# bowang-lab/BioReason

Hardware: NVIDIA H100
Metric: GRPO tokens/sec (rollout+update) (higher is better)
Workload: dtype bf16

## Files before the change

bioreason_b200/csrc/gemm_tc5.cu:

```cuda
#include "br_common.cuh"
#include "../../include/bioreason_b200.h"
#include "lora_dropout.cuh"
#include "wgmma.cuh"

namespace {

constexpr int BM = 128;
constexpr int BN = 128;
constexpr int BK = 64;
constexpr int NTHREADS = 288;

enum { MODE_STD = 0, MODE_LSE = 1, MODE_DLOGITS = 2 };

struct GemmParams {
    int M, N, K, K2;
    int ldd;
    void* D;
    const void* bias; int bias_f32;
    const bf16* residual; long long ldr;
    float alpha;
    int act;
    int out_f32;
    const int* row_map;
    bf16* aux; long long ld_aux;
    const int* target;
    float* pmax; float* psum; float* tgt_logit;
    const float* lse; const float* gscale;
    int n_tiles_m, n_tiles_n;
    int group_m;
    br::DropParams drop;
};

struct SmemLayout {
    static constexpr int A_BYTES = BM * BK * 2;
    static constexpr int B_BYTES = BN * BK * 2;
    static constexpr int STAGE_BYTES = A_BYTES + B_BYTES;
    static constexpr int NSTAGE = 6;
    static constexpr int TILE_BYTES = NSTAGE * STAGE_BYTES;
    static constexpr int TOTAL = TILE_BYTES + 256 + 1024;
};

__device__ __forceinline__ void tile_coords(int tile, int ntm, int ntn, int GROUP_M, int& mb, int& nb) {
    int per_group = GROUP_M * ntn;
    int g = tile / per_group;
    int first_m = g * GROUP_M;
    int gsize = min(GROUP_M, ntm - first_m);
    int r = tile - g * per_group;
    mb = first_m + (r % gsize);
    nb = r / gsize;
}

__device__ __forceinline__ float rbf(float x) { return __bfloat162float(__float2bfloat16(x)); }

__device__ __forceinline__ void masked_segment(float (&acc)[BN / 2], uint64_t adesc, uint64_t bdesc, int k0, int mb, int nb, int wg,
                                               const GemmParams& p) {
    const int lane = threadIdx.x & 31, q = lane & 3;
    const long long grow = p.drop.row0 + mb * BM + wg * 64 + ((threadIdx.x >> 5) & 3) * 16 + (lane >> 2);
    const int cg0 = (nb * BN) >> 3;
    br::wg_wait<0>();
    br::wg_fence_operand(acc);
    for (int kk = 0; kk < BK / 16;) {
        const int kc = k0 + 16 * kk;
        if (kc >= p.K2) break;
        const int jb = kc / p.drop.r;
        const int nk = min(p.drop.r - (kc - jb * p.drop.r), BK - 16 * kk) >> 4;
        float tmp[BN / 2];
#pragma unroll
        for (int i = 0; i < BN / 2; ++i) tmp[i] = 0.f;
        br::wg_fence();
        for (int t = 0; t < nk; ++t) br::wgmma_ss<BN>(tmp, adesc + 2 * (kk + t), bdesc + 2 * (kk + t), 1);
        br::wg_commit();
        br::wg_wait<0>();
        br::wg_fence_operand(tmp);
        const int j = p.drop.proj + jb;
#pragma unroll
        for (int set = 0; set < BN / 16; ++set) {
            uint32_t w[4];
            br::quad_words(br::drop_group(p.drop, grow + 8 * (q & 1), cg0 + 2 * set + (q >> 1), j), w);
#pragma unroll
            for (int g = 0; g < 4; ++g) {
                const int e = 4 * (2 * set + (g >> 1)) + 2 * (g & 1);
                acc[e] += br::keep_lo(w[g], p.drop.T) ? tmp[e] * p.drop.inv_keep : 0.f;
                acc[e + 1] += br::keep_hi(w[g], p.drop.T) ? tmp[e + 1] * p.drop.inv_keep : 0.f;
            }
        }
        kk += nk;
    }
}

template <int MODE, bool MASK>
__global__ void __launch_bounds__(NTHREADS, 1)
gemm_tc5_kernel(const __grid_constant__ CUtensorMap tmA, const __grid_constant__ CUtensorMap tmB,
                const __grid_constant__ CUtensorMap tmA2, const __grid_constant__ CUtensorMap tmB2,
                const GemmParams p) {
    using L = SmemLayout;
    extern __shared__ uint8_t smem_raw[];
    uint8_t* smem = reinterpret_cast<uint8_t*>((reinterpret_cast<uintptr_t>(smem_raw) + 1023) & ~uintptr_t(1023));
    uint64_t* full_bar = reinterpret_cast<uint64_t*>(smem + L::TILE_BYTES);
    uint64_t* empty_bar = full_bar + L::NSTAGE;

    const int warp = threadIdx.x >> 5;
    const int lane = threadIdx.x & 31;
    const int num_tiles = p.n_tiles_m * p.n_tiles_n;
    const int kb1 = (p.K + BK - 1) / BK;
    const int kb2 = (p.K2 + BK - 1) / BK;
    const int num_kb = kb1 + kb2;

    if (threadIdx.x == 0) {
        br::tma_prefetch_desc(&tmA);
        br::tma_prefetch_desc(&tmB);
        if (kb2) { br::tma_prefetch_desc(&tmA2); br::tma_prefetch_desc(&tmB2); }
        for (int s = 0; s < L::NSTAGE; ++s) { br::mbar_init(&full_bar[s], 1); br::mbar_init(&empty_bar[s], 2); }
        br::mbar_fence_init();
    }
    __syncthreads();

    if (warp == 8) {
        if (lane == 0) {
            int s = 0; uint32_t ph = 0;
            for (int tile = blockIdx.x; tile < num_tiles; tile += gridDim.x) {
                int mb, nb; tile_coords(tile, p.n_tiles_m, p.n_tiles_n, p.group_m, mb, nb);
                for (int kb = 0; kb < num_kb; ++kb) {
                    br::mbar_wait(&empty_bar[s], ph ^ 1);
                    uint8_t* sa = smem + s * L::STAGE_BYTES;
                    uint8_t* sb = sa + L::A_BYTES;
                    br::mbar_expect_tx(&full_bar[s], L::STAGE_BYTES);
                    if (kb < kb1) {
                        br::tma_load_2d(sa, &tmA, &full_bar[s], kb * BK, mb * BM);
                        br::tma_load_2d(sb, &tmB, &full_bar[s], kb * BK, nb * BN);
                    } else {
                        br::tma_load_2d(sa, &tmA2, &full_bar[s], (kb - kb1) * BK, mb * BM);
                        br::tma_load_2d(sb, &tmB2, &full_bar[s], (kb - kb1) * BK, nb * BN);
                    }
                    if (++s == L::NSTAGE) { s = 0; ph ^= 1; }
                }
            }
        }
        return;
    }
    const int wg = warp >> 2;
    const int wt = threadIdx.x & 127;
    int s = 0; uint32_t ph = 0;
    for (int tile = blockIdx.x; tile < num_tiles; tile += gridDim.x) {
        int mb, nb; tile_coords(tile, p.n_tiles_m, p.n_tiles_n, p.group_m, mb, nb);
        float acc[BN / 2];
#pragma unroll
        for (int i = 0; i < BN / 2; ++i) acc[i] = 0.f;
        int prev = 0;
        for (int kb = 0; kb < num_kb; ++kb) {
            br::mbar_wait(&full_bar[s], ph);
            const uint32_t sa = br::smem_u32(smem + s * L::STAGE_BYTES);
            const uint64_t adesc = br::wg_desc_k(sa + wg * 64 * 128);
            const uint64_t bdesc = br::wg_desc_k(sa + L::A_BYTES);
            if constexpr (MASK) {
                if (kb >= kb1) {
                    masked_segment(acc, adesc, bdesc, (kb - kb1) * BK, mb, nb, wg, p);
                    if (wt == 0) br::mbar_arrive(&empty_bar[prev]);
                    prev = s;
                    if (++s == L::NSTAGE) { s = 0; ph ^= 1; }
                    continue;
                }
            }
            br::wg_fence();
#pragma unroll
            for (int k = 0; k < BK / 16; ++k) br::wgmma_ss<BN>(acc, adesc + 2 * k, bdesc + 2 * k, 1);
            br::wg_commit();
            if (kb > 0) {
                br::wg_wait<1>();
                if (wt == 0) br::mbar_arrive(&empty_bar[prev]);
            }
            prev = s;
            if (++s == L::NSTAGE) { s = 0; ph ^= 1; }
        }
        br::wg_wait<0>();
        br::wg_fence_operand(acc);
        if (wt == 0) br::mbar_arrive(&empty_bar[prev]);

        const int r0 = mb * BM + wg * 64 + (warp & 3) * 16 + (lane >> 2);
        const int n0 = nb * BN;
        const int cq = 2 * (lane & 3);
        if constexpr (MODE == MODE_STD) {
#pragma unroll
            for (int hh = 0; hh < 2; ++hh) {
                const int row = r0 + 8 * hh;
                if (row >= p.M) continue;
                const long long orow = p.row_map ? (long long)p.row_map[row] : (long long)row;
                if (orow < 0) continue;
                float v[BN / 4];
#pragma unroll
                for (int i = 0; i < BN / 8; ++i) {
                    v[2 * i] = acc[4 * i + 2 * hh] * p.alpha;
                    v[2 * i + 1] = acc[4 * i + 2 * hh + 1] * p.alpha;
                    const int col = n0 + 8 * i + cq;
                    if (p.bias && n0 + 8 * i < p.N) {
                        if (p.bias_f32) {
                            const float* b = reinterpret_cast<const float*>(p.bias) + col;
                            v[2 * i] += __ldg(b); v[2 * i + 1] += __ldg(b + 1);
                        } else {
                            const bf16* b = reinterpret_cast<const bf16*>(p.bias) + col;
                            v[2 * i] += __bfloat162float(b[0]); v[2 * i + 1] += __bfloat162float(b[1]);
                        }
                    }
                }
                if (p.act == 1) {
#pragma unroll
                    for (int j = 0; j < BN / 16; ++j) {
                        if (n0 + 16 * j >= p.N) break;
                        if (p.aux) {
                            bf16* a = p.aux + orow * p.ld_aux + n0 + 16 * j + cq;
                            *reinterpret_cast<uint32_t*>(a) = br::pack_bf16(v[4 * j], v[4 * j + 1]);
                            *reinterpret_cast<uint32_t*>(a + 8) = br::pack_bf16(v[4 * j + 2], v[4 * j + 3]);
                        }
                        float o[2];
#pragma unroll
                        for (int e = 0; e < 2; ++e) {
                            const float g = rbf(v[4 * j + e]), u = rbf(v[4 * j + 2 + e]);
                            o[e] = rbf(g / (1.f + __expf(-g))) * u;
                        }
                        bf16* d = reinterpret_cast<bf16*>(p.D) + orow * (long long)p.ldd + (n0 >> 1) + 8 * j + cq;
                        *reinterpret_cast<uint32_t*>(d) = br::pack_bf16(o[0], o[1]);
                    }
                    continue;
                }
#pragma unroll
                for (int i = 0; i < BN / 8; ++i) {
                    if (n0 + 8 * i >= p.N) break;
                    const int col = n0 + 8 * i + cq;
                    float x0 = v[2 * i], x1 = v[2 * i + 1];
                    if (p.residual) {
                        const float2 r = br::unpack_bf16(__ldg(reinterpret_cast<const unsigned int*>(p.residual + orow * p.ldr + col)));
                        x0 = rbf(x0) + r.x; x1 = rbf(x1) + r.y;
                    }
                    if (p.out_f32) *reinterpret_cast<float2*>(reinterpret_cast<float*>(p.D) + orow * (long long)p.ldd + col) = make_float2(x0, x1);
                    else *reinterpret_cast<uint32_t*>(reinterpret_cast<bf16*>(p.D) + orow * (long long)p.ldd + col) = br::pack_bf16(x0, x1);
                }
            }
        } else if constexpr (MODE == MODE_LSE) {
#pragma unroll
            for (int hh = 0; hh < 2; ++hh) {
                const int row = r0 + 8 * hh;
                const bool row_ok = row < p.M;
                const int tgt = row_ok ? p.target[row] : -1;
                float mx = -INFINITY;
#pragma unroll
                for (int i = 0; i < BN / 8; ++i)
                    if (n0 + 8 * i < p.N) mx = fmaxf(mx, fmaxf(acc[4 * i + 2 * hh], acc[4 * i + 2 * hh + 1]) * p.alpha);
                mx = fmaxf(mx, __shfl_xor_sync(0xffffffffu, mx, 1));
                mx = fmaxf(mx, __shfl_xor_sync(0xffffffffu, mx, 2));
                float sm = 0.f;
#pragma unroll
                for (int i = 0; i < BN / 8; ++i) {
                    if (n0 + 8 * i >= p.N) continue;
                    const int col = n0 + 8 * i + cq;
                    const float x0 = acc[4 * i + 2 * hh] * p.alpha, x1 = acc[4 * i + 2 * hh + 1] * p.alpha;
                    sm += __expf(x0 - mx) + __expf(x1 - mx);
                    if (col == tgt) p.tgt_logit[row] = x0;
                    if (col + 1 == tgt) p.tgt_logit[row] = x1;
                }
                sm += __shfl_xor_sync(0xffffffffu, sm, 1);
                sm += __shfl_xor_sync(0xffffffffu, sm, 2);
                if (row_ok && (lane & 3) == 0) {
                    p.pmax[(long long)row * p.n_tiles_n + nb] = mx;
                    p.psum[(long long)row * p.n_tiles_n + nb] = sm;
                }
            }
        } else {
#pragma unroll
            for (int hh = 0; hh < 2; ++hh) {
                const int row = r0 + 8 * hh;
                if (row >= p.M) continue;
                const int tgt = p.target[row];
                const float lse = p.lse[row], gs = p.gscale[row];
#pragma unroll
                for (int i = 0; i < BN / 8; ++i) {
                    if (n0 + 8 * i >= p.N) break;
                    const int col = n0 + 8 * i + cq;
                    const float d0 = gs * ((col == tgt ? 1.f : 0.f) - __expf(acc[4 * i + 2 * hh] * p.alpha - lse));
                    const float d1 = gs * ((col + 1 == tgt ? 1.f : 0.f) - __expf(acc[4 * i + 2 * hh + 1] * p.alpha - lse));
                    *reinterpret_cast<uint32_t*>(reinterpret_cast<bf16*>(p.D) + (long long)row * p.ldd + col) = br::pack_bf16(d0, d1);
                }
            }
        }
    }
}

__global__ void lse_combine_kernel(const float* __restrict__ pmax, const float* __restrict__ psum, const float* __restrict__ tgt_logit,
                                   const int* __restrict__ target, int M, int nt, float* __restrict__ lse, float* __restrict__ logp) {
    int row = blockIdx.x * (blockDim.x >> 5) + (threadIdx.x >> 5);
    if (row >= M) return;
    int lane = threadIdx.x & 31;
    float mx = -INFINITY;
    for (int t = lane; t < nt; t += 32) mx = fmaxf(mx, pmax[(long long)row * nt + t]);
    mx = br::warp_max(mx);
    float s = 0.f;
    for (int t = lane; t < nt; t += 32) s += psum[(long long)row * nt + t] * __expf(pmax[(long long)row * nt + t] - mx);
    s = br::warp_sum(s);
    if (lane == 0) {
        float l = logf(s) + mx;
        if (lse) lse[row] = l;
        if (logp) logp[row] = (target[row] >= 0) ? tgt_logit[row] - l : 0.f;
    }
}

typedef CUresult (*PFN_encodeTiled)(CUtensorMap*, CUtensorMapDataType, cuuint32_t, void*, const cuuint64_t*, const cuuint64_t*,
                                    const cuuint32_t*, const cuuint32_t*, CUtensorMapInterleave, CUtensorMapSwizzle,
                                    CUtensorMapL2promotion, CUtensorMapFloatOOBfill);
PFN_encodeTiled get_encode() {
    static PFN_encodeTiled fn = nullptr;
    if (!fn) {
        void* f = nullptr;
        cudaDriverEntryPointQueryResult q;
        if (cudaGetDriverEntryPoint("cuTensorMapEncodeTiled", &f, cudaEnableDefault, &q) == cudaSuccess && q == cudaDriverEntryPointSuccess)
            fn = reinterpret_cast<PFN_encodeTiled>(f);
    }
    return fn;
}

template <int MODE, bool MASK = false>
int launch(const CUtensorMap& a, const CUtensorMap& b, const CUtensorMap& a2, const CUtensorMap& b2, const GemmParams& p, cudaStream_t st) {
    auto kern = gemm_tc5_kernel<MODE, MASK>;
    static bool attr_set = false;
    if (!attr_set) {
        BR_CHECK_CUDA(cudaFuncSetAttribute(kern, cudaFuncAttributeMaxDynamicSharedMemorySize, SmemLayout::TOTAL));
        attr_set = true;
    }
    int tiles = p.n_tiles_m * p.n_tiles_n;
    int grid = tiles < br_num_sms() ? tiles : br_num_sms();
    kern<<<grid, NTHREADS, SmemLayout::TOTAL, st>>>(a, b, a2, b2, p);
    BR_CHECK_LAUNCH();
    return BR_OK;
}

int run_gemm(int mode, const void* A, int64_t lda, const void* B, int64_t ldb, int M, int N, int K, const void* A2, int64_t lda2,
             const void* B2, int64_t ldb2, int K2, GemmParams& p, cudaStream_t st, bool masked = false) {
    BR_CHECK_ARG(M > 0 && N > 0 && K > 0, "gemm: empty problem M=%d N=%d K=%d", M, N, K);
    BR_CHECK_ARG(N % 8 == 0 && K % 8 == 0 && lda % 8 == 0 && ldb % 8 == 0, "gemm: N, K, lda, ldb must be multiples of 8");
    BR_CHECK_ARG(((uintptr_t)A % 16 == 0) && ((uintptr_t)B % 16 == 0), "gemm: operands must be 16-byte aligned");
    p.M = M; p.N = N; p.K = K; p.K2 = (A2 && B2) ? K2 : 0;
    p.n_tiles_m = (M + BM - 1) / BM;
    p.n_tiles_n = (N + BN - 1) / BN;
    {
        const long long a_block = (long long)BM * (K + p.K2) * 2;
        long long g = (16ll << 20) / (a_block > 0 ? a_block : 1);
        if (g < 8) g = 8;
        if (g > p.n_tiles_m) g = p.n_tiles_m;
        p.group_m = (int)g;
    }
    CUtensorMap ta, tb, ta2, tb2;
    int rc;
    if ((rc = br_make_tmap_2d_bf16(&ta, A, M, K, lda, BM))) return rc;
    if ((rc = br_make_tmap_2d_bf16(&tb, B, N, K, ldb, BN))) return rc;
    if (p.K2) {
        BR_CHECK_ARG(K2 % 8 == 0 && lda2 % 8 == 0 && ldb2 % 8 == 0, "gemm: K2, lda2, ldb2 must be multiples of 8");
        if ((rc = br_make_tmap_2d_bf16(&ta2, A2, M, K2, lda2, BM))) return rc;
        if ((rc = br_make_tmap_2d_bf16(&tb2, B2, N, K2, ldb2, BN))) return rc;
    } else { ta2 = ta; tb2 = tb; }
    if (masked) return launch<MODE_STD, true>(ta, tb, ta2, tb2, p, st);
    if (mode == MODE_STD) return launch<MODE_STD>(ta, tb, ta2, tb2, p, st);
    if (mode == MODE_LSE) return launch<MODE_LSE>(ta, tb, ta2, tb2, p, st);
    return launch<MODE_DLOGITS>(ta, tb, ta2, tb2, p, st);
}

}

int br_make_tmap_2d_bf16(CUtensorMap* out, const void* base, uint64_t rows, uint64_t cols, uint64_t ld_elems, uint32_t box_rows) {
    PFN_encodeTiled enc = get_encode();
    if (!enc) { br_set_error("cuTensorMapEncodeTiled not available from the driver"); return BR_ERR_CUDA; }
    cuuint64_t gdim[2] = {cols, rows};
    cuuint64_t gstr[1] = {ld_elems * 2};
    cuuint32_t box[2] = {64, box_rows};
    cuuint32_t estr[2] = {1, 1};
    CUresult r = enc(out, CU_TENSOR_MAP_DATA_TYPE_BFLOAT16, 2, const_cast<void*>(base), gdim, gstr, box, estr, CU_TENSOR_MAP_INTERLEAVE_NONE,
                     CU_TENSOR_MAP_SWIZZLE_128B, CU_TENSOR_MAP_L2_PROMOTION_L2_256B, CU_TENSOR_MAP_FLOAT_OOB_FILL_NONE);
    if (r != CUDA_SUCCESS) {
        br_set_error("cuTensorMapEncodeTiled failed (%d) rows=%llu cols=%llu ld=%llu box_rows=%u base=%p", (int)r, (unsigned long long)rows,
                     (unsigned long long)cols, (unsigned long long)ld_elems, box_rows, base);
        return BR_ERR_CUDA;
    }
    return BR_OK;
}

extern "C" {

int br_gemm_bf16(const void* A, int64_t lda, const void* B, int64_t ldb, void* D, int64_t ldd, int M, int N, int K,
                 const br_gemm_epilogue* e, void* stream) {
    GemmParams p;
    memset(&p, 0, sizeof(p));
    p.D = D; p.ldd = (int)ldd; p.alpha = 1.f;
    const void *A2 = nullptr, *B2 = nullptr; int64_t lda2 = 0, ldb2 = 0; int K2 = 0;
    bool masked = false;
    if (e) {
        p.bias = e->bias; p.bias_f32 = e->bias_dtype == BR_F32;
        p.residual = reinterpret_cast<const bf16*>(e->residual); p.ldr = e->ldr;
        p.alpha = e->alpha; p.act = e->act; p.out_f32 = e->out_dtype == BR_F32;
        p.row_map = e->row_map; p.aux = reinterpret_cast<bf16*>(e->aux_out); p.ld_aux = e->ld_aux;
        A2 = e->A2; B2 = e->B2; lda2 = e->lda2; ldb2 = e->ldb2; K2 = e->K2;
        BR_CHECK_ARG(!(p.act == 1 && (p.out_f32 || p.residual)), "gemm: gated-SiLU epilogue writes bf16 without residual");
        BR_CHECK_ARG(!(p.act == 1 && N % 16 != 0), "gemm: gated-SiLU epilogue needs N %% 16 == 0");
        if (e->lora_dropout) {
            int rc;
            if ((rc = br::check_drop(e->lora_dropout, "gemm"))) return rc;
            const int r = e->lora_dropout->r;
            BR_CHECK_ARG(A2 && B2 && r % 16 == 0 && r > 0 && K2 % r == 0 && e->lora_dropout->proj + K2 / r <= 8,
                         "gemm: masked LoRA segment needs A2/B2 with K2 = n_proj * r, r %% 16 == 0 (K2=%d r=%d)", K2, r);
            BR_CHECK_ARG(!p.row_map, "gemm: masked LoRA segment indexes mask rows by input row; no row_map");
            p.drop = br::drop_params(*e->lora_dropout);
            masked = true;
        }
    }
    BR_CHECK_ARG(ldd % 8 == 0 && (uintptr_t)D % 16 == 0, "gemm: D must be 16-byte aligned with ldd %% 8 == 0");
    return run_gemm(MODE_STD, A, lda, B, ldb, M, N, K, A2, lda2, B2, ldb2, K2, p, (cudaStream_t)stream, masked);
}

int64_t br_lmhead_workspace_bytes(int M, int V) {
    int nt = (V + 127) / 128;
    return (int64_t)M * nt * 2 * sizeof(float) + (int64_t)M * sizeof(float);
}

int br_lmhead_logprob_fwd(const void* H, int64_t ldh, const void* W, int64_t ldw, const int32_t* target, int M, int V, int K, float scale,
                          float* logp, float* lse, void* workspace, void* stream) {
    GemmParams p;
    memset(&p, 0, sizeof(p));
    int nt_max = (V + 127) / 128;
    p.alpha = scale; p.target = target;
    p.pmax = reinterpret_cast<float*>(workspace);
    p.psum = p.pmax + (int64_t)M * nt_max;
    p.tgt_logit = p.psum + (int64_t)M * nt_max;
    cudaStream_t st = (cudaStream_t)stream;
    BR_CHECK_CUDA(cudaMemsetAsync(p.tgt_logit, 0, (size_t)M * sizeof(float), st));
    int rc = run_gemm(MODE_LSE, H, ldh, W, ldw, M, V, K, nullptr, 0, nullptr, 0, 0, p, st);
    if (rc) return rc;
    const int wpb = 8;
    lse_combine_kernel<<<(M + wpb - 1) / wpb, wpb * 32, 0, st>>>(p.pmax, p.psum, p.tgt_logit, target, M, p.n_tiles_n, lse, logp);
    BR_CHECK_LAUNCH();
    return BR_OK;
}

int br_lmhead_dlogits(const void* H, int64_t ldh, const void* W, int64_t ldw, const int32_t* target, const float* lse, const float* gscale,
                      int M, int V, int K, float scale, void* dlogits, int64_t ldd, void* stream) {
    GemmParams p;
    memset(&p, 0, sizeof(p));
    p.alpha = scale; p.target = target; p.lse = lse; p.gscale = gscale; p.D = dlogits; p.ldd = (int)ldd;
    BR_CHECK_ARG(ldd % 8 == 0, "lmhead_dlogits: ldd %% 8");
    return run_gemm(MODE_DLOGITS, H, ldh, W, ldw, M, V, K, nullptr, 0, nullptr, 0, 0, p, (cudaStream_t)stream);
}

}
```

bioreason_b200/csrc/wgmma.cuh:

```cuda
#pragma once
#include <stdint.h>

namespace br {

__device__ __forceinline__ uint64_t wg_desc_k(uint32_t smem_addr) {
    return (uint64_t)((smem_addr & 0x3FFFF) >> 4) | ((uint64_t)1 << 16) | ((uint64_t)(1024 >> 4) << 32) | ((uint64_t)1 << 62);
}
__device__ __forceinline__ uint64_t wg_desc_mn(uint32_t smem_addr, uint32_t lbo, uint32_t sbo) {
    return (uint64_t)((smem_addr & 0x3FFFF) >> 4) | ((uint64_t)((lbo >> 4) & 0x3FFF) << 16) | ((uint64_t)((sbo >> 4) & 0x3FFF) << 32) |
           ((uint64_t)1 << 62);
}
__device__ __forceinline__ void wg_fence() { asm volatile("wgmma.fence.sync.aligned;" ::: "memory"); }
__device__ __forceinline__ void wg_commit() { asm volatile("wgmma.commit_group.sync.aligned;" ::: "memory"); }
template <int N>
__device__ __forceinline__ void wg_wait() { asm volatile("wgmma.wait_group.sync.aligned %0;" ::"n"(N) : "memory"); }
template <int N>
__device__ __forceinline__ void wg_fence_operand(float (&d)[N]) {
#pragma unroll
    for (int i = 0; i < N; ++i) asm volatile("" : "+f"(d[i])::"memory");
}

#define BR_WG_F8(i) "+f"(d[i]), "+f"(d[i + 1]), "+f"(d[i + 2]), "+f"(d[i + 3]), "+f"(d[i + 4]), "+f"(d[i + 5]), "+f"(d[i + 6]), "+f"(d[i + 7])
#define BR_WG_F16(i) BR_WG_F8(i), BR_WG_F8(i + 8)
#define BR_WG_F32(i) BR_WG_F16(i), BR_WG_F16(i + 16)
#define BR_WG_F64(i) BR_WG_F32(i), BR_WG_F32(i + 32)

template <int N, int TA, int TB> struct WgSS;
template <int N, int TB> struct WgRS;

template <int TA, int TB> struct WgSS<16, TA, TB> {
    static __device__ __forceinline__ void run(float (&d)[8], uint64_t a, uint64_t b, int accumulate) {
        asm volatile("{\n.reg .pred p;\nsetp.ne.b32 p, %10, 0;\n"
                     "wgmma.mma_async.sync.aligned.m64n16k16.f32.bf16.bf16 {%0, %1, %2, %3, %4, %5, %6, %7}, %8, %9, p, 1, 1, %11, %12;\n}\n"
                     : BR_WG_F8(0) : "l"(a), "l"(b), "r"(accumulate), "n"(TA), "n"(TB));
    }
};
template <int TA, int TB> struct WgSS<32, TA, TB> {
    static __device__ __forceinline__ void run(float (&d)[16], uint64_t a, uint64_t b, int accumulate) {
        asm volatile("{\n.reg .pred p;\nsetp.ne.b32 p, %18, 0;\n"
                     "wgmma.mma_async.sync.aligned.m64n32k16.f32.bf16.bf16 {%0, %1, %2, %3, %4, %5, %6, %7, %8, %9, %10, %11, %12, %13, %14, %15}, %16, %17, p, 1, 1, %19, %20;\n}\n"
                     : BR_WG_F16(0) : "l"(a), "l"(b), "r"(accumulate), "n"(TA), "n"(TB));
    }
};
template <int TA, int TB> struct WgSS<64, TA, TB> {
    static __device__ __forceinline__ void run(float (&d)[32], uint64_t a, uint64_t b, int accumulate) {
        asm volatile("{\n.reg .pred p;\nsetp.ne.b32 p, %34, 0;\n"
                     "wgmma.mma_async.sync.aligned.m64n64k16.f32.bf16.bf16 {%0, %1, %2, %3, %4, %5, %6, %7, %8, %9, %10, %11, %12, %13, %14, %15, %16, %17, %18, %19, %20, %21, %22, %23, %24, %25, %26, %27, %28, %29, %30, %31}, %32, %33, p, 1, 1, %35, %36;\n}\n"
                     : BR_WG_F32(0) : "l"(a), "l"(b), "r"(accumulate), "n"(TA), "n"(TB));
    }
};
template <int TA, int TB> struct WgSS<128, TA, TB> {
    static __device__ __forceinline__ void run(float (&d)[64], uint64_t a, uint64_t b, int accumulate) {
        asm volatile("{\n.reg .pred p;\nsetp.ne.b32 p, %66, 0;\n"
                     "wgmma.mma_async.sync.aligned.m64n128k16.f32.bf16.bf16 {%0, %1, %2, %3, %4, %5, %6, %7, %8, %9, %10, %11, %12, %13, %14, %15, %16, %17, %18, %19, %20, %21, %22, %23, %24, %25, %26, %27, %28, %29, %30, %31, %32, %33, %34, %35, %36, %37, %38, %39, %40, %41, %42, %43, %44, %45, %46, %47, %48, %49, %50, %51, %52, %53, %54, %55, %56, %57, %58, %59, %60, %61, %62, %63}, %64, %65, p, 1, 1, %67, %68;\n}\n"
                     : BR_WG_F64(0) : "l"(a), "l"(b), "r"(accumulate), "n"(TA), "n"(TB));
    }
};
template <int TB> struct WgRS<16, TB> {
    static __device__ __forceinline__ void run(float (&d)[8], const uint32_t (&a)[4], uint64_t b, int accumulate) {
        asm volatile("{\n.reg .pred p;\nsetp.ne.b32 p, %13, 0;\n"
                     "wgmma.mma_async.sync.aligned.m64n16k16.f32.bf16.bf16 {%0, %1, %2, %3, %4, %5, %6, %7}, {%8, %9, %10, %11}, %12, p, 1, 1, %14;\n}\n"
                     : BR_WG_F8(0) : "r"(a[0]), "r"(a[1]), "r"(a[2]), "r"(a[3]), "l"(b), "r"(accumulate), "n"(TB));
    }
};
template <int TB> struct WgRS<32, TB> {
    static __device__ __forceinline__ void run(float (&d)[16], const uint32_t (&a)[4], uint64_t b, int accumulate) {
        asm volatile("{\n.reg .pred p;\nsetp.ne.b32 p, %21, 0;\n"
                     "wgmma.mma_async.sync.aligned.m64n32k16.f32.bf16.bf16 {%0, %1, %2, %3, %4, %5, %6, %7, %8, %9, %10, %11, %12, %13, %14, %15}, {%16, %17, %18, %19}, %20, p, 1, 1, %22;\n}\n"
                     : BR_WG_F16(0) : "r"(a[0]), "r"(a[1]), "r"(a[2]), "r"(a[3]), "l"(b), "r"(accumulate), "n"(TB));
    }
};
template <int TB> struct WgRS<64, TB> {
    static __device__ __forceinline__ void run(float (&d)[32], const uint32_t (&a)[4], uint64_t b, int accumulate) {
        asm volatile("{\n.reg .pred p;\nsetp.ne.b32 p, %37, 0;\n"
                     "wgmma.mma_async.sync.aligned.m64n64k16.f32.bf16.bf16 {%0, %1, %2, %3, %4, %5, %6, %7, %8, %9, %10, %11, %12, %13, %14, %15, %16, %17, %18, %19, %20, %21, %22, %23, %24, %25, %26, %27, %28, %29, %30, %31}, {%32, %33, %34, %35}, %36, p, 1, 1, %38;\n}\n"
                     : BR_WG_F32(0) : "r"(a[0]), "r"(a[1]), "r"(a[2]), "r"(a[3]), "l"(b), "r"(accumulate), "n"(TB));
    }
};
template <int TB> struct WgRS<128, TB> {
    static __device__ __forceinline__ void run(float (&d)[64], const uint32_t (&a)[4], uint64_t b, int accumulate) {
        asm volatile("{\n.reg .pred p;\nsetp.ne.b32 p, %69, 0;\n"
                     "wgmma.mma_async.sync.aligned.m64n128k16.f32.bf16.bf16 {%0, %1, %2, %3, %4, %5, %6, %7, %8, %9, %10, %11, %12, %13, %14, %15, %16, %17, %18, %19, %20, %21, %22, %23, %24, %25, %26, %27, %28, %29, %30, %31, %32, %33, %34, %35, %36, %37, %38, %39, %40, %41, %42, %43, %44, %45, %46, %47, %48, %49, %50, %51, %52, %53, %54, %55, %56, %57, %58, %59, %60, %61, %62, %63}, {%64, %65, %66, %67}, %68, p, 1, 1, %70;\n}\n"
                     : BR_WG_F64(0) : "r"(a[0]), "r"(a[1]), "r"(a[2]), "r"(a[3]), "l"(b), "r"(accumulate), "n"(TB));
    }
};
#undef BR_WG_F8
#undef BR_WG_F16
#undef BR_WG_F32
#undef BR_WG_F64

template <int N, int TA = 0, int TB = 0>
__device__ __forceinline__ void wgmma_ss(float (&d)[N / 2], uint64_t a, uint64_t b, int accumulate) { WgSS<N, TA, TB>::run(d, a, b, accumulate); }
template <int N, int TB = 0>
__device__ __forceinline__ void wgmma_rs(float (&d)[N / 2], const uint32_t (&a)[4], uint64_t b, int accumulate) { WgRS<N, TB>::run(d, a, b, accumulate); }

}
```

Baseline: 1181.

## Add 256-wide N tiles with m64n256 wgmma for large unmasked GEMMs

Templates the persistent TMA/wgmma GEMM on tile width and adds a 128x256 tile variant using m64n256k16 wgmma with 4 pipeline stages. The wide tile is picked for unmasked GEMMs with N>=256, K>=512 and enough tiles to fill the SMs twice over. The aim is to raise arithmetic intensity per loaded A tile and cut wgmma issue overhead. In exchange the accumulator grows to 128 fp32 registers per thread, which adds register pressure with a risk of spills, and the pipeline is shallower. The LSE epilogue is split into 128-column halves so its partial-max/sum layout stays the same.

```diff
diff --git a/bioreason_b200/csrc/gemm_tc5.cu b/bioreason_b200/csrc/gemm_tc5.cu
--- a/bioreason_b200/csrc/gemm_tc5.cu
+++ b/bioreason_b200/csrc/gemm_tc5.cu
@@ -6,7 +6,6 @@
 namespace {
 
 constexpr int BM = 128;
-constexpr int BN = 128;
 constexpr int BK = 64;
 constexpr int NTHREADS = 288;
 
@@ -31,11 +30,12 @@
     br::DropParams drop;
 };
 
+template <int BN>
 struct SmemLayout {
     static constexpr int A_BYTES = BM * BK * 2;
     static constexpr int B_BYTES = BN * BK * 2;
     static constexpr int STAGE_BYTES = A_BYTES + B_BYTES;
-    static constexpr int NSTAGE = 6;
+    static constexpr int NSTAGE = BN == 128 ? 6 : 4;
     static constexpr int TILE_BYTES = NSTAGE * STAGE_BYTES;
     static constexpr int TOTAL = TILE_BYTES + 256 + 1024;
 };
@@ -52,6 +52,7 @@
 
 __device__ __forceinline__ float rbf(float x) { return __bfloat162float(__float2bfloat16(x)); }
 
+template <int BN>
 __device__ __forceinline__ void masked_segment(float (&acc)[BN / 2], uint64_t adesc, uint64_t bdesc, int k0, int mb, int nb, int wg,
                                                const GemmParams& p) {
     const int lane = threadIdx.x & 31, q = lane & 3;
@@ -88,12 +89,15 @@
     }
 }
 
-template <int MODE, bool MASK>
+template <int BN, int MODE, bool MASK>
 __global__ void __launch_bounds__(NTHREADS, 1)
 gemm_tc5_kernel(const __grid_constant__ CUtensorMap tmA, const __grid_constant__ CUtensorMap tmB,
                 const __grid_constant__ CUtensorMap tmA2, const __grid_constant__ CUtensorMap tmB2,
                 const GemmParams p) {
-    using L = SmemLayout;
+    static_assert(BN == 128 || BN == 256, "tile width");
+    static_assert(!MASK || BN == 128, "the masked LoRA segment runs on 128-wide tiles");
+    constexpr int NSUB = BN / 128;
+    using L = SmemLayout<BN>;
     extern __shared__ uint8_t smem_raw[];
     uint8_t* smem = reinterpret_cast<uint8_t*>((reinterpret_cast<uintptr_t>(smem_raw) + 1023) & ~uintptr_t(1023));
     uint64_t* full_bar = reinterpret_cast<uint64_t*>(smem + L::TILE_BYTES);
@@ -101,7 +105,7 @@
 
     const int warp = threadIdx.x >> 5;
     const int lane = threadIdx.x & 31;
-    const int num_tiles = p.n_tiles_m * p.n_tiles_n;
+    const int num_tiles = p.n_tiles_m * ((p.n_tiles_n + NSUB - 1) / NSUB);
     const int kb1 = (p.K + BK - 1) / BK;
     const int kb2 = (p.K2 + BK - 1) / BK;
     const int num_kb = kb1 + kb2;
@@ -119,7 +123,7 @@
         if (lane == 0) {
             int s = 0; uint32_t ph = 0;
             for (int tile = blockIdx.x; tile < num_tiles; tile += gridDim.x) {
-                int mb, nb; tile_coords(tile, p.n_tiles_m, p.n_tiles_n, p.group_m, mb, nb);
+                int mb, nb; tile_coords(tile, p.n_tiles_m, (p.n_tiles_n + NSUB - 1) / NSUB, p.group_m, mb, nb);
                 for (int kb = 0; kb < num_kb; ++kb) {
                     br::mbar_wait(&empty_bar[s], ph ^ 1);
                     uint8_t* sa = smem + s * L::STAGE_BYTES;
@@ -142,7 +146,7 @@
     const int wt = threadIdx.x & 127;
     int s = 0; uint32_t ph = 0;
     for (int tile = blockIdx.x; tile < num_tiles; tile += gridDim.x) {
-        int mb, nb; tile_coords(tile, p.n_tiles_m, p.n_tiles_n, p.group_m, mb, nb);
+        int mb, nb; tile_coords(tile, p.n_tiles_m, (p.n_tiles_n + NSUB - 1) / NSUB, p.group_m, mb, nb);
         float acc[BN / 2];
 #pragma unroll
         for (int i = 0; i < BN / 2; ++i) acc[i] = 0.f;
@@ -154,7 +158,7 @@
             const uint64_t bdesc = br::wg_desc_k(sa + L::A_BYTES);
             if constexpr (MASK) {
                 if (kb >= kb1) {
-                    masked_segment(acc, adesc, bdesc, (kb - kb1) * BK, mb, nb, wg, p);
+                    masked_segment<BN>(acc, adesc, bdesc, (kb - kb1) * BK, mb, nb, wg, p);
                     if (wt == 0) br::mbar_arrive(&empty_bar[prev]);
                     prev = s;
                     if (++s == L::NSTAGE) { s = 0; ph ^= 1; }
@@ -237,31 +241,36 @@
             }
         } else if constexpr (MODE == MODE_LSE) {
 #pragma unroll
-            for (int hh = 0; hh < 2; ++hh) {
-                const int row = r0 + 8 * hh;
-                const bool row_ok = row < p.M;
-                const int tgt = row_ok ? p.target[row] : -1;
-                float mx = -INFINITY;
-#pragma unroll
-                for (int i = 0; i < BN / 8; ++i)
-                    if (n0 + 8 * i < p.N) mx = fmaxf(mx, fmaxf(acc[4 * i + 2 * hh], acc[4 * i + 2 * hh + 1]) * p.alpha);
-                mx = fmaxf(mx, __shfl_xor_sync(0xffffffffu, mx, 1));
-                mx = fmaxf(mx, __shfl_xor_sync(0xffffffffu, mx, 2));
-                float sm = 0.f;
-#pragma unroll
-                for (int i = 0; i < BN / 8; ++i) {
-                    if (n0 + 8 * i >= p.N) continue;
-                    const int col = n0 + 8 * i + cq;
-                    const float x0 = acc[4 * i + 2 * hh] * p.alpha, x1 = acc[4 * i + 2 * hh + 1] * p.alpha;
-                    sm += __expf(x0 - mx) + __expf(x1 - mx);
-                    if (col == tgt) p.tgt_logit[row] = x0;
-                    if (col + 1 == tgt) p.tgt_logit[row] = x1;
-                }
-                sm += __shfl_xor_sync(0xffffffffu, sm, 1);
-                sm += __shfl_xor_sync(0xffffffffu, sm, 2);
-                if (row_ok && (lane & 3) == 0) {
-                    p.pmax[(long long)row * p.n_tiles_n + nb] = mx;
-                    p.psum[(long long)row * p.n_tiles_n + nb] = sm;
+            for (int h = 0; h < NSUB; ++h) {
+                const int nh = n0 + 128 * h;
+                if (NSUB > 1 && nh >= p.N) break;
+#pragma unroll
+                for (int hh = 0; hh < 2; ++hh) {
+                    const int row = r0 + 8 * hh;
+                    const bool row_ok = row < p.M;
+                    const int tgt = row_ok ? p.target[row] : -1;
+                    float mx = -INFINITY;
+#pragma unroll
+                    for (int i = 0; i < 16; ++i)
+                        if (nh + 8 * i < p.N) mx = fmaxf(mx, fmaxf(acc[64 * h + 4 * i + 2 * hh], acc[64 * h + 4 * i + 2 * hh + 1]) * p.alpha);
+                    mx = fmaxf(mx, __shfl_xor_sync(0xffffffffu, mx, 1));
+                    mx = fmaxf(mx, __shfl_xor_sync(0xffffffffu, mx, 2));
+                    float sm = 0.f;
+#pragma unroll
+                    for (int i = 0; i < 16; ++i) {
+                        if (nh + 8 * i >= p.N) continue;
+                        const int col = nh + 8 * i + cq;
+                        const float x0 = acc[64 * h + 4 * i + 2 * hh] * p.alpha, x1 = acc[64 * h + 4 * i + 2 * hh + 1] * p.alpha;
+                        sm += __expf(x0 - mx) + __expf(x1 - mx);
+                        if (col == tgt) p.tgt_logit[row] = x0;
+                        if (col + 1 == tgt) p.tgt_logit[row] = x1;
+                    }
+                    sm += __shfl_xor_sync(0xffffffffu, sm, 1);
+                    sm += __shfl_xor_sync(0xffffffffu, sm, 2);
+                    if (row_ok && (lane & 3) == 0) {
+                        p.pmax[(long long)row * p.n_tiles_n + nb * NSUB + h] = mx;
+                        p.psum[(long long)row * p.n_tiles_n + nb * NSUB + h] = sm;
+                    }
                 }
             }
         } else {
@@ -316,19 +325,27 @@
     return fn;
 }
 
-template <int MODE, bool MASK = false>
+template <int BN, int MODE, bool MASK = false>
 int launch(const CUtensorMap& a, const CUtensorMap& b, const CUtensorMap& a2, const CUtensorMap& b2, const GemmParams& p, cudaStream_t st) {
-    auto kern = gemm_tc5_kernel<MODE, MASK>;
+    auto kern = gemm_tc5_kernel<BN, MODE, MASK>;
     static bool attr_set = false;
     if (!attr_set) {
-        BR_CHECK_CUDA(cudaFuncSetAttribute(kern, cudaFuncAttributeMaxDynamicSharedMemorySize, SmemLayout::TOTAL));
+        BR_CHECK_CUDA(cudaFuncSetAttribute(kern, cudaFuncAttributeMaxDynamicSharedMemorySize, SmemLayout<BN>::TOTAL));
         attr_set = true;
     }
-    int tiles = p.n_tiles_m * p.n_tiles_n;
+    int tiles = p.n_tiles_m * ((p.n_tiles_n + BN / 128 - 1) / (BN / 128));
     int grid = tiles < br_num_sms() ? tiles : br_num_sms();
-    kern<<<grid, NTHREADS, SmemLayout::TOTAL, st>>>(a, b, a2, b2, p);
+    kern<<<grid, NTHREADS, SmemLayout<BN>::TOTAL, st>>>(a, b, a2, b2, p);
     BR_CHECK_LAUNCH();
     return BR_OK;
+}
+
+template <int BN>
+int launch_mode(int mode, const CUtensorMap& a, const CUtensorMap& b, const CUtensorMap& a2, const CUtensorMap& b2, const GemmParams& p,
+                cudaStream_t st) {
+    if (mode == MODE_STD) return launch<BN, MODE_STD>(a, b, a2, b2, p, st);
+    if (mode == MODE_LSE) return launch<BN, MODE_LSE>(a, b, a2, b2, p, st);
+    return launch<BN, MODE_DLOGITS>(a, b, a2, b2, p, st);
 }
 
 int run_gemm(int mode, const void* A, int64_t lda, const void* B, int64_t ldb, int M, int N, int K, const void* A2, int64_t lda2,
@@ -338,7 +355,9 @@
     BR_CHECK_ARG(((uintptr_t)A % 16 == 0) && ((uintptr_t)B % 16 == 0), "gemm: operands must be 16-byte aligned");
     p.M = M; p.N = N; p.K = K; p.K2 = (A2 && B2) ? K2 : 0;
     p.n_tiles_m = (M + BM - 1) / BM;
-    p.n_tiles_n = (N + BN - 1) / BN;
+    p.n_tiles_n = (N + 127) / 128;
+    const bool wide = !masked && N >= 256 && K >= 512 && (long long)p.n_tiles_m * ((N + 255) / 256) >= 2ll * br_num_sms();
+    const int bn = wide ? 256 : 128;
     {
         const long long a_block = (long long)BM * (K + p.K2) * 2;
         long long g = (16ll << 20) / (a_block > 0 ? a_block : 1);
@@ -349,16 +368,14 @@
     CUtensorMap ta, tb, ta2, tb2;
     int rc;
     if ((rc = br_make_tmap_2d_bf16(&ta, A, M, K, lda, BM))) return rc;
-    if ((rc = br_make_tmap_2d_bf16(&tb, B, N, K, ldb, BN))) return rc;
+    if ((rc = br_make_tmap_2d_bf16(&tb, B, N, K, ldb, bn))) return rc;
     if (p.K2) {
         BR_CHECK_ARG(K2 % 8 == 0 && lda2 % 8 == 0 && ldb2 % 8 == 0, "gemm: K2, lda2, ldb2 must be multiples of 8");
         if ((rc = br_make_tmap_2d_bf16(&ta2, A2, M, K2, lda2, BM))) return rc;
-        if ((rc = br_make_tmap_2d_bf16(&tb2, B2, N, K2, ldb2, BN))) return rc;
+        if ((rc = br_make_tmap_2d_bf16(&tb2, B2, N, K2, ldb2, bn))) return rc;
     } else { ta2 = ta; tb2 = tb; }
-    if (masked) return launch<MODE_STD, true>(ta, tb, ta2, tb2, p, st);
-    if (mode == MODE_STD) return launch<MODE_STD>(ta, tb, ta2, tb2, p, st);
-    if (mode == MODE_LSE) return launch<MODE_LSE>(ta, tb, ta2, tb2, p, st);
-    return launch<MODE_DLOGITS>(ta, tb, ta2, tb2, p, st);
+    if (masked) return launch<128, MODE_STD, true>(ta, tb, ta2, tb2, p, st);
+    return wide ? launch_mode<256>(mode, ta, tb, ta2, tb2, p, st) : launch_mode<128>(mode, ta, tb, ta2, tb2, p, st);
 }
 
 }
diff --git a/bioreason_b200/csrc/wgmma.cuh b/bioreason_b200/csrc/wgmma.cuh
--- a/bioreason_b200/csrc/wgmma.cuh
+++ b/bioreason_b200/csrc/wgmma.cuh
@@ -24,6 +24,7 @@
 #define BR_WG_F16(i) BR_WG_F8(i), BR_WG_F8(i + 8)
 #define BR_WG_F32(i) BR_WG_F16(i), BR_WG_F16(i + 16)
 #define BR_WG_F64(i) BR_WG_F32(i), BR_WG_F32(i + 32)
+#define BR_WG_F128(i) BR_WG_F64(i), BR_WG_F64(i + 64)
 
 template <int N, int TA, int TB> struct WgSS;
 template <int N, int TB> struct WgRS;
@@ -54,6 +55,13 @@
         asm volatile("{\n.reg .pred p;\nsetp.ne.b32 p, %66, 0;\n"
                      "wgmma.mma_async.sync.aligned.m64n128k16.f32.bf16.bf16 {%0, %1, %2, %3, %4, %5, %6, %7, %8, %9, %10, %11, %12, %13, %14, %15, %16, %17, %18, %19, %20, %21, %22, %23, %24, %25, %26, %27, %28, %29, %30, %31, %32, %33, %34, %35, %36, %37, %38, %39, %40, %41, %42, %43, %44, %45, %46, %47, %48, %49, %50, %51, %52, %53, %54, %55, %56, %57, %58, %59, %60, %61, %62, %63}, %64, %65, p, 1, 1, %67, %68;\n}\n"
                      : BR_WG_F64(0) : "l"(a), "l"(b), "r"(accumulate), "n"(TA), "n"(TB));
+    }
+};
+template <int TA, int TB> struct WgSS<256, TA, TB> {
+    static __device__ __forceinline__ void run(float (&d)[128], uint64_t a, uint64_t b, int accumulate) {
+        asm volatile("{\n.reg .pred p;\nsetp.ne.b32 p, %130, 0;\n"
+                     "wgmma.mma_async.sync.aligned.m64n256k16.f32.bf16.bf16 {%0, %1, %2, %3, %4, %5, %6, %7, %8, %9, %10, %11, %12, %13, %14, %15, %16, %17, %18, %19, %20, %21, %22, %23, %24, %25, %26, %27, %28, %29, %30, %31, %32, %33, %34, %35, %36, %37, %38, %39, %40, %41, %42, %43, %44, %45, %46, %47, %48, %49, %50, %51, %52, %53, %54, %55, %56, %57, %58, %59, %60, %61, %62, %63, %64, %65, %66, %67, %68, %69, %70, %71, %72, %73, %74, %75, %76, %77, %78, %79, %80, %81, %82, %83, %84, %85, %86, %87, %88, %89, %90, %91, %92, %93, %94, %95, %96, %97, %98, %99, %100, %101, %102, %103, %104, %105, %106, %107, %108, %109, %110, %111, %112, %113, %114, %115, %116, %117, %118, %119, %120, %121, %122, %123, %124, %125, %126, %127}, %128, %129, p, 1, 1, %131, %132;\n}\n"
+                     : BR_WG_F128(0) : "l"(a), "l"(b), "r"(accumulate), "n"(TA), "n"(TB));
     }
 };
 template <int TB> struct WgRS<16, TB> {
@@ -88,6 +96,7 @@
 #undef BR_WG_F16
 #undef BR_WG_F32
 #undef BR_WG_F64
+#undef BR_WG_F128
 
 template <int N, int TA = 0, int TB = 0>
 __device__ __forceinline__ void wgmma_ss(float (&d)[N / 2], uint64_t a, uint64_t b, int accumulate) { WgSS<N, TA, TB>::run(d, a, b, accumulate); }
```

After: 1222 (median of 6 runs). 1.03x the previous value.
